# AMReX-Fluids/IAMR

Hardware: AMD Instinct MI355X
Metric: cells-advanced/sec (higher is better)
Workload: dtype f64; 1 GPU; TaylorGreen 3D single level, one 256^3 box per GPU in a 1x1x1 arrangement (256x256x256 cells), periodic, nu=1e-4 cfl=0.7 Godunov_PLM be_cn_theta=0.5, full NavierStokes::advance per step

## Files before the change

### iamr_amd/csrc/diffusion.hip

```cpp
#include "operators.h"
#include "launch.h"

namespace iamrx {

void scale_by(MultiFab& y, const MultiFab& x, int xcomp, int ng, bool divide);

namespace {
void scale_comp(MultiFab& y, int ycomp, const MultiFab& x, int xcomp, int ng, bool divide)
{
    const FabD *yt = y.d_tab, *xt = x.d_tab;
    for_each(*y.layout, cell_type(), ng, Context::get().stream, [=] __device__(int i, int j, int k, int f) {
        const double x = xt[f](i, j, k, xcomp);
        if (!divide) yt[f](i, j, k, ycomp) *= x;
        else if (x != 0.0 || yt[f](i, j, k, ycomp) != 0.0) yt[f](i, j, k, ycomp) /= x;
    });
}
void crse_soln(MultiFab& out, const MultiFab& Sc, int sigma, int rho_comp, bool over_rho)
{
    out.define(Sc.layout, cell_type(), 1, 0);
    MultiFab::Copy(out, Sc, sigma, 0, 1, 0);
    if (over_rho) scale_comp(out, 0, Sc, rho_comp, 0, true);
}
}

// ... 82 lines not shown
    MultiFab Rhs(layout, cell_type(), 3, 0);
    const bool want_flux = tflux != nullptr && tflux[0] != nullptr;
    TensorFlux fx{{want_flux ? tflux[0] : nullptr, want_flux ? tflux[1] : nullptr, want_flux ? tflux[2] : nullptr}, 0.0, false};
    if (want_flux) for (int d = 0; d < 3; ++d) tflux[d]->setVal(0.0);
    MultiFab cdata;
    TensorCF cf{&cdata, crse ? crse->cgeom : nullptr, crse ? crse->ratio : 2};
    const bool from_visc = theta != 1.0 && !want_flux && visc_old_term;
    if (!from_visc && theta != 1.0) {
        IAMRX_ASSERT(U_old && U_old->ngrow >= 1);
        MultiFab Soln0(layout, cell_type(), 3, 1);
        MultiFab::Copy(Soln0, *U_old, Xvel, 0, 3, 1);
        if (crse) { cdata.define(crse->crse_old->layout, cell_type(), 3, 0); MultiFab::Copy(cdata, *crse->crse_old, Xvel, 0, 3, 0); }
        fx.fac = 1.0 - theta; fx.add = false;
        tensor_apply(g, Rhs, Soln0, 0.0, -(1.0 - theta) * dt, nullptr, eta_n, bc_visc, 3, crse ? &cf : nullptr, want_flux ? &fx : nullptr);
    } else if (!from_visc) Rhs.setVal(0.0);
    {
        const FabD *nt = U_new.d_tab, *ot = U_old ? U_old->d_tab : nullptr, *rt = Rhs.d_tab, *ht = rho_half.d_tab;
        const FabD* vt = from_visc ? visc_old_term->d_tab : nullptr;
        const double va = (1.0 - theta) * dt;
        const bool mom = rho_flag == 3;
        IAMRX_ASSERT(!mom || ot);
        for_each(*layout, cell_type(), 0, Context::get().stream, [=] __device__(int i, int j, int k, int f) {
            const double r = mom ? ot[f](i, j, k, rho_comp) : ht[f](i, j, k, 0);
            for (int n = 0; n < 3; ++n) {
                const double un = nt[f](i, j, k, n) * r;
                nt[f](i, j, k, n) = un;
                double rr;
                if (vt) { const double v = vt[f](i, j, k, n); rr = va * v + 0.0 * v; }
                else rr = rt[f](i, j, k, n);
                rt[f](i, j, k, n) = rr + un;
            }
        });
    }
    double avg = 0.0;
    double rn3[3];
    Rhs.norm0_comps(0, 3, 0, rn3);
    for (int n = 0; n < 3; ++n) avg += (1.0 / 3.0) * rn3[n];
    const double tol_abs = visc_tol * avg;
    if (fill_new) fill_new(U_new);
    MultiFab Soln, acoef;
    Soln.view_of(U_new, Xvel, 3);
    if (rho_flag == 3) acoef.view_of(U_new, rho_comp, 1);
    else acoef.view_of(rho_half, 0, 1);
    MGOpts vo = o;
    vo.maxorder = 2;
    if (crse) { cdata.define(crse->crse_new->layout, cell_type(), 3, 0); MultiFab::Copy(cdata, *crse->crse_new, Xvel, 0, 3, 0); }
    fx.fac = theta; fx.add = true;
    MGStats st = tensor_solve(g, Soln, Rhs, 1.0, theta * dt, &acoef, eta_np1, bc_visc, 3, visc_tol, tol_abs, vo, crse ? &cf : nullptr, want_flux ? &fx : nullptr);
    return st;
}

// ... 59 lines not shown
```

### iamr_amd/csrc/k_abec.hip

```cpp
#include "kernels.h"
#include "launch.h"
#include <map>
#include <array>
#include <cstring>
#include <vector>
#include <algorithm>

namespace iamrx {

struct CfC1 { double c1[3][3]; double c2[3][3], c3[3][3]; int maxorder; int maintain; };

__device__ __forceinline__ void cf_maintain(const FabD& phi, const FabD& cfm, const BoxD& b, const CfC1& t, int i, int j, int k, double pnew)
{
    const int idx[3] = {i, j, k};
    for (int d = 0; d < 3; ++d) {
        const int NX = min(b.len(d) + 1, t.maxorder);
        if (NX < 2) continue;
        const int target = NX == 2 ? 1 : 2;
        for (int side = 0; side < 2; ++side) {
            const int s = side == 0 ? 1 : -1, f = side == 0 ? b.lo[d] : b.hi[d];
            if ((idx[d] - f) * s + 1 != target) continue;
            int g[3] = {i, j, k};
            g[d] = f - s;
            if (cfm(g[0], g[1], g[2]) != 1.0) continue;
// ... 860 lines not shown
    }
    return true;
}

static bool abec_sig_on() { return tune("ABEC_SIG", 1) != 0; }

AbecLevel abec_level(const AbecCoef& c, const MultiFab& phi, int rhs_ngrow, int nbc, const DomainBC* bcs, bool has_cf, bool finest)
{
    AbecLevel lv;
    const Layout& l = *phi.layout;
    lv.boxes = &l.boxes; lv.nlocal = l.nlocal();
    for (int d = 0; d < 3; ++d) lv.max_len[d] = l.max_len[d];
    lv.ncomp = phi.ncomp; lv.phi_ngrow = phi.ngrow; lv.rhs_ngrow = rhs_ngrow;
    lv.sig = c.sig != nullptr; lv.sig_ngrow = c.sig ? c.sig->ngrow : 0;
    lv.has_a = c.a && c.alpha != 0.0; lv.a_ngrow = c.a ? c.a->ngrow : 0;
    lv.b_uniform = c.b_uniform != 0; lv.tensor_eta = c.tensor_eta != 0; lv.tensor = c.tensor != 0; lv.b_ncomp = c.b[0]->ncomp;
    lv.nbc = nbc; lv.bcs = bcs; lv.has_cf = has_cf; lv.finest = finest;
    return lv;
}

static bool rb_shape_ok(const BoxD& b, int nx) { return (nx == 128 || nx == 256) && b.len(0) == nx && b.len(1) >= 16 && b.len(2) >= 16; }
static bool rb_walls_covered(const Geometry& g, const AbecLevel& lv)
{
    if (g.periodic[0] && g.periodic[1] && g.periodic[2]) return true;
    if (!lv.bcs || lv.nbc < 1) return false;
    for (int n = 0; n < lv.ncomp; ++n) { RbBC r; if (!rb_make_bc(g, lv.bcs[n < lv.nbc ? n : 0], r)) return false; }
    return true;
}
static bool box_spans(const Geometry& g, const BoxD& b, int min_len)
{
    for (int d = 0; d < 3; ++d) if (b.lo[d] != g.domain.lo[d] || b.hi[d] != g.domain.hi[d] || b.len(d) < min_len) return false;
// ... 1572 lines not shown
        const FabD fa = ft[f], ca = ct[f];
        const int c[3] = {i, j, k};
        for (int n = 0; n < nc; ++n) {
            double s = 0.0;
            for (int rb = 0; rb < 2; ++rb)
                for (int ra = 0; ra < 2; ++ra) {
                    int q[3];
                    q[dir] = 2 * c[dir]; q[da] = 2 * c[da] + ra; q[db] = 2 * c[db] + rb;
                    s += fa(q[0], q[1], q[2], n);
                }
            ca(i, j, k, n) = s * 0.25;
        }
    });
}

void abec_flux(const Geometry& g, const AbecCoef& c, const MultiFab& phi, MultiFab* const flux[3], MultiFab* const add_to[3])
{
    if (phi.nlocal() == 0) return;
    const FabD* pt = phi.d_tab;
    const int nc = phi.ncomp;
    for (int d = 0; d < 3; ++d) {
        const double fac = c.beta / g.dx[d];
        const FabD* bt = c.b[d]->d_tab;
        const int bnc = c.b[d]->ncomp;
        const FabD* ft = flux && flux[d] ? flux[d]->d_tab : nullptr;
        const FabD* ut = add_to && add_to[d] ? add_to[d]->d_tab : nullptr;
        for_each(*phi.layout, face_type(d), 0, Context::get().stream, [=] __device__(int i, int j, int k, int f) {
            const FabD p = pt[f], b = bt[f];
            int m[3] = {i, j, k}; m[d] -= 1;
            for (int n = 0; n < nc; ++n) {
// ... 4 lines not shown
        });
    }
}

void mac_divergence(const Geometry& g, MultiFab& div, const MultiFab* const umac[3])
{
    if (div.nlocal() == 0) return;
    const FabD *dt = div.d_tab, *ut = umac[0]->d_tab, *vt = umac[1]->d_tab, *wt = umac[2]->d_tab;
    const double dx = g.dx[0], dy = g.dx[1], dz = g.dx[2];
    for_each(*div.layout, cell_type(), 0, Context::get().stream, [=] __device__(int i, int j, int k, int f) {
        const FabD u = ut[f], v = vt[f], w = wt[f];
        dt[f](i, j, k, 0) = (u(i + 1, j, k) - u(i, j, k)) / dx + (v(i, j + 1, k) - v(i, j, k)) / dy + (w(i, j, k + 1) - w(i, j, k)) / dz;
    });
}

void mac_rhs(const Geometry& g, MultiFab& rhs, const MultiFab* const umac[3], const MultiFab* S)
{
    if (rhs.nlocal() == 0) return;
    const FabD *rt = rhs.d_tab, *ut = umac[0]->d_tab, *vt = umac[1]->d_tab, *wt = umac[2]->d_tab;
    const FabD* st = S ? S->d_tab : nullptr;
    const double dx = g.dx[0], dy = g.dx[1], dz = g.dx[2];
    for_each(*rhs.layout, cell_type(), 0, Context::get().stream, [=] __device__(int i, int j, int k, int f) {
        const FabD u = ut[f], v = vt[f], w = wt[f];
        const double div = (u(i + 1, j, k) - u(i, j, k)) / dx + (v(i, j + 1, k) - v(i, j, k)) / dy + (w(i, j, k + 1) - w(i, j, k)) / dz;
        double r = -div;
        if (st) r += st[f](i, j, k, 0);
        rt[f](i, j, k, 0) = r;
    });
}

void mac_bcoef(MultiFab* const b[3], const MultiFab& rho, int rho_comp, double scale)
{
    if (rho.nlocal() == 0) return;
    const FabD* rt = rho.d_tab;
    for (int d = 0; d < 3; ++d) {
        const FabD* bt = b[d]->d_tab;
        for_each(*rho.layout, face_type(d), 0, Context::get().stream, [=] __device__(int i, int j, int k, int f) {
            const FabD r = rt[f];
            int m[3] = {i, j, k}; m[d] -= 1;
            const double rf = 0.5 * (r(m[0], m[1], m[2], rho_comp) + r(i, j, k, rho_comp));
            bt[f](i, j, k, 0) = scale / rf;
        });
    }
}
// ... 29 lines not shown
```

### iamr_amd/csrc/k_basic.hip

```cpp
#include "kernels.h"
#include "launch.h"
#include <algorithm>

namespace iamrx {

__global__ void __launch_bounds__(256) k_fill(double* __restrict__ p, size_t n, double v)
{
    size_t i = (size_t)blockIdx.x * 256 + threadIdx.x;
    const size_t stride = (size_t)gridDim.x * 256;
    for (; i < n; i += stride) p[i] = v;
}

void launch_fill(double* p, size_t n, double v, hipStream_t s)
{
    if (n == 0) return;
    size_t nb = (n + 255) / 256;
    if (nb > 4096) nb = 4096;
    hipLaunchKernelGGL(k_fill, dim3((unsigned)nb), dim3(256), 0, s, p, n, v);
}

__global__ void __launch_bounds__(256) k_copy_plan(const CopyDesc* __restrict__ descs, const FabD* __restrict__ src,
                                                   const FabD* __restrict__ dst, int scomp, int dcomp, int nc, int add)
{
    const CopyDesc cd = descs[blockIdx.y];
// ... 507 lines not shown
    for_each_2ph(*y.layout, y.type, ng, nc, Context::get().stream,
        [=] __device__(int i, int j, int k, int f, int n) { return yt[f](i, j, k, ycomp + n) + a * xt[f](i, j, k, xcomp + n); },
        [=] __device__(int i, int j, int k, int f, int n, double v) { yt[f](i, j, k, ycomp + n) = v; });
}

void mf_add_scalar(MultiFab& y, double a, int comp, int nc, int ng)
{
    if (!y.base) return;
    const FabD* yt = y.d_tab;
    for_each(*y.layout, y.type, ng, Context::get().stream, [=] __device__(int i, int j, int k, int f) {
        const FabD yy = yt[f];
        for (int n = 0; n < nc; ++n) yy(i, j, k, comp + n) += a;
    });
}

void mf_mult(MultiFab& y, double a, int comp, int nc, int ng)
{
    trace_blas_site("mult", y.layout ? y.layout->local_cells() * nc : 0);
    if (!y.base) return;
    const FabD* yt = y.d_tab;
    for_each_2ph(*y.layout, y.type, ng, nc, Context::get().stream,
        [=] __device__(int i, int j, int k, int f, int n) { return yt[f](i, j, k, comp + n) * a; },
        [=] __device__(int i, int j, int k, int f, int n, double v) { yt[f](i, j, k, comp + n) = v; });
}

__global__ void __launch_bounds__(256) k_mult_shell(const BoxD* __restrict__ boxes, const FabD* __restrict__ yt, int t0, int t1, int t2, int ng, int comp, int nc, double a)
{
    const int fab = blockIdx.y;
    BoxD b = boxes[fab];
    b.hi[0] += t0; b.hi[1] += t1; b.hi[2] += t2;
// ... 145 lines not shown
```

### iamr_amd/csrc/kernels.h

```cpp
#pragma once
#include "core.h"
#include "mf.h"

namespace iamrx {

void launch_fill(double* p, size_t n, double v, hipStream_t s);
void launch_copy_plan(const CopyDesc* d, int nd, long maxpts, const FabD* src, const FabD* dst, int scomp, int dcomp, int nc, hipStream_t s, bool add = false);
void launch_pack(const CopyDesc* d, int nd, long maxpts, const FabD* src, double* buf, long pts_total, int scomp, int nc, hipStream_t s);
void launch_unpack(const CopyDesc* d, int nd, long maxpts, const FabD* dst, const double* buf, long pts_total, int dcomp, int nc, hipStream_t s, bool add = false);
void launch_copy_plan_w(const CopyDesc* d, const int2* w, int nw, const FabD* src, const FabD* dst, int scomp, int dcomp, int nc, hipStream_t s, bool add);
void launch_pack_w(const CopyDesc* d, const int2* w, int nw, const FabD* src, double* buf, long pts_total, int scomp, int nc, hipStream_t s);
void launch_unpack_w(const CopyDesc* d, const int2* w, int nw, const FabD* dst, const double* buf, long pts_total, int dcomp, int nc, hipStream_t s, bool add);
double reduce_norm0(const MultiFab& mf, int comp, int nc, int ng, bool global = false);
void reduce_norm0_comps(const MultiFab& mf, int comp, int nc, int ng, double* out, bool global = false);
void reduce_minmax(const MultiFab& mf, int comp, int ng, double& mn, double& mx, bool global = true);
double reduce_sum_unique(const MultiFab& mf, int comp, const Geometry& g, bool global = false);
void reduce_sum_integrated(const MultiFab& S, int rho_comp, int trac_comp, const MultiFab* cov, double out[3]);
constexpr int SUM_COMPS_MAX = 8;
void reduce_sum_comps(const MultiFab& mf, int n, const int* comps, const MultiFab* cov, double* out);
void reduce_dots(int nout, const MultiFab* const* x, const MultiFab* const* y, int comp, int nc, const Geometry& g, double* out, bool local = false);
void reduce_dots_dev(int nout, const MultiFab* const* x, const MultiFab* const* y, int comp, int nc, const Geometry& g, double* d_out, bool local = false);
enum { PROBE_NODAL_GS4 = 0, PROBE_ABEC_GSRB = 1, PROBE_GOD_Z = 2, PROBE_PRED_Z = 3, PROBE_COUNT = 4 };
void kernel_probe_start(int which, long min_points, int stride);
void kernel_probe_stop(int which, double* total_ms, long* launches);
void kernel_probes_pause(bool on);
bool kernel_probe_begin(int which, long points);
void kernel_probe_end(int which);
void gs4_probe_start(long min_nodes, int stride);
void gs4_probe_stop(double* total_ms, long* launches);
void mf_lincomb(MultiFab& dst, double a, const MultiFab& x, double b, const MultiFab& y, int comp, int nc, int ng);
void mf_saxpy(MultiFab& y, double a, const MultiFab& x, int xcomp, int ycomp, int nc, int ng);
void mf_add_scalar(MultiFab& y, double a, int comp, int nc, int ng);
void mf_mult(MultiFab& y, double a, int comp, int nc, int ng);
void mf_mult_ghosts(MultiFab& y, double a, int comp, int nc, int ng);
void dense_check_cover(const char* who, const Geometry& g, const Layout& lay);
void dense_pack(const Geometry& g, const MultiFab& S, int comp, double* dst, bool cplx);
void dense_pack_imag(const Geometry& g, const MultiFab& S, int comp, double* dst);
void dense_gather(const Geometry& g, const MultiFab& S, int comp, double* R);
bool dense_needs_gather(const MultiFab& S);
void dense_unpack(const Geometry& g, MultiFab& S, int comp, const double* src, double scale);

void stats_accumulate(MultiFab& avg, const MultiFab& S, int vcomp, double dt_avg, double t_sum, bool fluct);
void stats_derive_vel_avg(MultiFab& out, int ocomp, const MultiFab& avg, double t_mean, double t_fluct);

constexpr int PROFILE_NQ = 14;
struct ProfileLevel { const MultiFab* S; const MultiFab* cov; const Geometry* g; };
int profile_nbins(const Geometry& g0, int dir, int bin_level);
// ... 179 lines not shown
bool abec_gsrb_rb_cf_ok(const Geometry& g, const AbecCoef& c, const MultiFab& phi);
bool abec_gsrb_rb_nbr_ok(const Geometry& g, const AbecCoef& c, const MultiFab& phi, const MultiFab& rhs, int nbc, const DomainBC* bcs);
bool abec_gsrb_rb_nbr_level_ok(const Geometry& g, const Layout& l, int ncomp, bool sig_form, bool has_a, int nbc, const DomainBC* bcs);
void abec_gsrb_fused(const Geometry& g, const AbecCoef& c, const MultiFab& phi_in, MultiFab& phi_out, const MultiFab& rhs, double omega,
                     const DomainBC* bcs, int nbc);
void abec_residual(const Geometry& g, const AbecCoef& c, MultiFab& out, const MultiFab& phi, const MultiFab* rhs, double* norm_out = nullptr);
bool abec_bottom_device_ok(const Geometry& g, const Layout& l, const DomainBC* bcs, int nbc, int ncomp, bool cf = false);
void abec_bottom_solve(const Geometry& g, const AbecCoef& c, MultiFab& cor, const MultiFab& res, const DomainBC& bc, bool singular,
                       double eps_rel, int maxiter, int nub, int nuf, double omega, int* d_iters, const CfTab* cftab = nullptr);
void abec_apply_domain_bc(const Geometry& g, MultiFab& phi, const DomainBC& bc, bool inhomog, const MultiFab* bcval, int comp0 = 0, int ncomp = -1);
void abec_apply_domain_bc_percomp(const Geometry& g, MultiFab& phi, const DomainBC* bcs, int ncomp, bool inhomog, const MultiFab* bcval);
void cc_restrict(MultiFab& crse, const MultiFab& fine);
void cc_prolong_add(MultiFab& fine, const MultiFab& crse);
void face_avgdown(MultiFab& crse, const MultiFab& fine, int dir);
void abec_flux(const Geometry& g, const AbecCoef& c, const MultiFab& phi, MultiFab* const flux[3], MultiFab* const add_to[3]);
void mac_rhs(const Geometry& g, MultiFab& rhs, const MultiFab* const umac[3], const MultiFab* S);
void mac_bcoef(MultiFab* const b[3], const MultiFab& rho, int rho_comp, double scale);
void mac_divergence(const Geometry& g, MultiFab& div, const MultiFab* const umac[3]);

void godunov_extrap_vel_to_faces(const Geometry& g, const MultiFab& vel, const MultiFab* force, MultiFab* const umac[3],
                                 double dt, const BCRec* bc, bool use_forces_in_trans, int scheme = 0);
void godunov_compute_aofs(const Geometry& g, MultiFab& aofs, int acomp, const MultiFab& S, int ncomp, const MultiFab* force,
                          const MultiFab* divu, MultiFab* const umac[3], const int* iconserv, double dt, const BCRec* bc,
                          bool is_velocity, bool use_forces_in_trans, MultiFab* const edge_out[3], MultiFab* const flux_out[3], int scheme = 0);


struct NodalImages { bool on = false; int refl = 0; };
bool nodal_residual(const Geometry& g, MultiFab& out, const MultiFab& x, const MultiFab& sig, const MultiFab* rhs, double* norm_out = nullptr,
                    const NodalImages& img = NodalImages());
void nodal_gs_color(const Geometry& g, MultiFab& x, const MultiFab& rhs, const MultiFab& sig, int color, const MultiFab* dmask = nullptr);
struct NodalLevel {
    const std::vector<BoxD>* boxes = nullptr;
// ... 66 lines not shown
```

### iamr_amd/csrc/macproj.hip

```cpp
#include "operators.h"
#include "launch.h"

namespace iamrx {

LayoutP merged_solve_layout(const Geometry& g, const LayoutP& l)
{
    if (!l || l->replicated || l->total_cells() != g.domain.npts()) return nullptr;
    LayoutP ml = coalesce_layout(l);
    return (ml->id != l->id && ml->boxes.size() < l->boxes.size()) ? ml : nullptr;
}

MGStats mlmg_mac_solve(const Geometry& g, MultiFab* const umac[3], const MultiFab& rho, int rho_comp, const MultiFab* S,
                       MultiFab& mac_phi, double rhs_scale, const DomainBC& bc, double mac_tol, double mac_abs_tol,
                       const MGOpts& opts, MultiFab* const fluxes[3], const MultiFab* cphi, const Geometry* cgeom, int ratio)
{
    LayoutP layout = mac_phi.layout;
    if (!cgeom) {
        if (LayoutP ml = merged_solve_layout(g, layout)) {
            MultiFab um_m[3], fl_m[3], rho_m(ml, cell_type(), 1, std::min(rho.ngrow, 1)), phi_m(ml, cell_type(), 1, mac_phi.ngrow), S_m;
            MultiFab *ump[3], *flp[3];
            for (int d = 0; d < 3; ++d) {
                um_m[d].define(ml, face_type(d), 1, 0); relayout_copy(um_m[d], *umac[d], 1); ump[d] = &um_m[d];
                if (fluxes) { fl_m[d].define(ml, face_type(d), 1, 0); flp[d] = &fl_m[d]; }
            }
            relayout_copy(rho_m, rho, 1, rho_comp, 0);
            relayout_copy(phi_m, mac_phi, 1);
            if (S) { S_m.define(ml, cell_type(), 1, 0); relayout_copy(S_m, *S, 1); }
            MGStats st = mlmg_mac_solve(g, ump, rho_m, 0, S ? &S_m : nullptr, phi_m, rhs_scale, bc, mac_tol, mac_abs_tol, opts, fluxes ? flp : nullptr,
                                        nullptr, nullptr, ratio);
            relayout_copy(mac_phi, phi_m, 1);
            for (int d = 0; d < 3; ++d) { relayout_copy(*umac[d], um_m[d], 1); if (fluxes) relayout_copy(*fluxes[d], fl_m[d], 1); }
            return st;
        }
    }
    MultiFab bcoef[3];
    MultiFab* bp[3];
    const MultiFab* bcp[3];
    for (int d = 0; d < 3; ++d) { bcoef[d].define(layout, face_type(d), 1, 0); bp[d] = &bcoef[d]; bcp[d] = &bcoef[d]; }
    mac_bcoef(bp, rho, rho_comp, 1.0 / rhs_scale);

    MultiFab rhs(layout, cell_type(), 1, 0);
    const MultiFab* um[3] = {umac[0], umac[1], umac[2]};
    mac_rhs(g, rhs, um, S);

    CellMG mg(g, layout, 1, bc, opts);
    mg.setScalars(0.0, 1.0);
    mg.setBCoeffs(bcp);
    if (rho.ngrow >= 1) mg.setBCoeffsFromCell(&rho, rho_comp, 1.0 / rhs_scale);
    if (cgeom) mg.setCoarseFineBC(cphi, *cgeom, ratio);
    mg.prepare();
    MGStats st = mg.solve(mac_phi, rhs, mac_tol, mac_abs_tol);
    mg.fluxes(mac_phi, fluxes, umac);
    return st;
}

MGStats mac_sync_solve(const Geometry& g, FluxRegister& mr, const MultiFab& rho_half, double dt, LayoutP fine_layout, int ratio,
                       MultiFab* const Ucorr[3], MultiFab& mac_sync_phi, const DomainBC& bc, double tol, double abs_tol, const MGOpts& opts,
                       const Geometry* cgeom, int cratio)
{
    LayoutP layout = mac_sync_phi.layout;
    MultiFab Rhs(layout, cell_type(), 1, 0);
    Rhs.setVal(0.0);
    mr.Reflux(Rhs, g.dx[0] * g.dx[1] * g.dx[2], -1.0, 0, 0, 1);
    {
        MultiFab fz(fine_layout, cell_type(), 1, 0);
        fz.setVal(0.0);
// ... 14 lines not shown
```

### iamr_amd/csrc/mf.h

```cpp
#pragma once
#include <functional>
#include "core.h"
#include <vector>
#include <memory>
#include <map>
#include <array>

namespace iamrx {

enum class ReduceOp { Sum, Max, Min };

struct Message {
    int peer;
    double* dev_ptr;
    size_t count;
};

struct Comm {
    int rank = 0, nranks = 1;
    virtual ~Comm() = default;
    virtual void allreduce(double* host_vals, int n, ReduceOp op) { (void)host_vals; (void)n; (void)op; }
    virtual void allreduce_device(double* dev_vals, int n, ReduceOp op, hipStream_t s) { (void)dev_vals; (void)n; (void)op; (void)s; }
    virtual void exchange(const std::vector<Message>& sends, const std::vector<Message>& recvs, hipStream_t s)
    {
// ... 64 lines not shown
    void mark() { IAMRX_ASSERT(next < ev.size()); IAMRX_HIP_CHECK(hipEventRecord(ev[next++], Context::get().stream)); }
    static void mark(PassTimer* t) { if (t) t->mark(); }
    void finish(float* ms)
    {
        IAMRX_ASSERT(next == ev.size());
        IAMRX_HIP_CHECK(hipEventSynchronize(ev.back()));
        for (size_t q = 0; q + 1 < ev.size(); ++q) IAMRX_HIP_CHECK(hipEventElapsedTime(&ms[q], ev[q], ev[q + 1]));
        next = 0;
    }
};

double tune(const char* key, double dflt);
double tune_by_name(const char* key, double dflt);
void trace_blas_site(const char* what, long points);
void tuning_set(const char* key, double value);
void tuning_load_environment();

struct ProfScope {
    static bool enabled;
    bool on;
    std::string key;
    double t0 = 0.0;
    explicit ProfScope(const char* name);
    ~ProfScope();
};
#define PROF_NEXT(var, name) do { (var).reset(); (var) = std::make_unique<::iamrx::ProfScope>(name); } while (0)
void scope_profile_enable(bool on, bool reset);
std::string scope_profile_report();

void register_layout_evictor(std::function<void(uint64_t)> f);
// ... 144 lines not shown
```

### iamr_amd/csrc/mf.hip

```cpp
#include "mf.h"
#include <climits>
#include <array>
#include <execinfo.h>
#include <dlfcn.h>
#include <chrono>
#include <functional>
#include <tuple>
#include "launch.h"
#include "kernels.h"
#include <algorithm>
#include <cstring>
#include <atomic>

namespace iamrx {

Context& Context::get()
{
    static Context c;
    return c;
}

void Context::init(int dev)
{
    tuning_load_environment();
// ... 209 lines not shown
{
    size_t i = ((uintptr_t)key >> 2) & (kTuneSlots - 1);
    for (int probe = 0; probe < 16; ++probe, i = (i + 1) & (kTuneSlots - 1)) {
        TuneSlot& t = g_tune_slots[i];
        if (t.key == key && t.ver == g_tune_version) return t.set ? t.val : dflt;
        if (t.key == nullptr || t.ver != g_tune_version) {
            auto& m = tuning_map();
            auto it = m.find(key);
            t.key = key; t.ver = g_tune_version; t.set = it != m.end(); t.val = t.set ? it->second : 0.0;
            return t.set ? t.val : dflt;
        }
    }
    return tune_by_name(key, dflt);
}
void tuning_set(const char* key, double value) { tuning_map()[key] = value; ++g_tune_version; }

bool ProfScope::enabled = false;
namespace {
struct ScopeStat { double ms = 0.0; long calls = 0; };
std::map<std::string, ScopeStat>& scope_stats() { static auto* m = new std::map<std::string, ScopeStat>(); return *m; }
std::vector<std::string>& scope_stack() { static auto* v = new std::vector<std::string>(); return *v; }
double now_ms() { return std::chrono::duration<double, std::milli>(std::chrono::steady_clock::now().time_since_epoch()).count(); }
}
ProfScope::ProfScope(const char* name) : on(enabled)
{
    if (!on) return;
    auto& st = scope_stack();
    key = st.empty() ? std::string(name) : st.back() + "/" + name;
    st.push_back(key);
    Context::get().sync();
// ... 888 lines not shown
```

### iamr_amd/csrc/mlmg.h

```cpp
#pragma once
#include <functional>
#include "mf.h"
#include "kernels.h"
#include <vector>
#include <memory>

namespace iamrx {

inline bool mg_stalled_at_floor(const std::vector<double>& hist, double r0, double target, bool fast)
{
    const size_t n = hist.size();
    if (n == 0 || !(hist[n - 1] <= 10.0 * target)) return false;
    if (n >= 4 && hist[n - 1] > 0.9 * hist[n - 4]) return true;
    if (!fast || n < 2) return false;
    const double last = hist[n - 1] / hist[n - 2];
    double best = 1.0, prev = r0;
    for (size_t i = 0; i + 1 < n; ++i) { if (prev > 0.0) best = std::min(best, hist[i] / prev); prev = hist[i]; }
    return last > 0.5 && best < 0.2;
}


struct MGOpts {
    int nu1 = 2, nu2 = 2, nuf = 8, nub = 0;
    int max_iters = 200;
// ... 77 lines not shown

class CellMG {
public:
    CellMG(const Geometry& g, LayoutP layout, int ncomp, const DomainBC& bc, const MGOpts& o);
    void setScalars(double alpha, double beta) { m_alpha = alpha; m_beta = beta; }
    void setACoeffs(const MultiFab* a) { m_a0 = a; }
    void setBCoeffs(const MultiFab* const b[3]) { for (int d = 0; d < 3; ++d) m_b0[d] = b[d]; }
    void setBCoeffsFromCell(const MultiFab* sig, int comp, double scale) { m_sig = sig; m_sig_comp = comp; m_sig_scale = scale; }
    void setTensor(bool t) { m_tensor = t; }
    void setTensorEta(bool t) { m_tensor_eta = t; }
    void setDomainBCs(const DomainBC* bcs, int n) { m_bcn.assign(bcs, bcs + n); }
    void setCoarseFineBC(const MultiFab* crse, const Geometry& cgeom, int ratio) { m_cf = true; m_crse = crse; m_cgeom = cgeom; m_ratio = ratio; }
    void prepare();
    void prepareBoundary();
    void fillBoundaryData(MultiFab& phi);
    MGStats solve(MultiFab& phi, const MultiFab& rhs, double rtol, double atol);
    void apply(MultiFab& out, MultiFab& phi);
    void fluxes(MultiFab& phi, MultiFab* const flux[3], MultiFab* const add_to[3]);
    int nlevels() const { return (int)m_lev.size(); }
    AbecCoef coef(int l) const;
    AbecCoef smoother_coef(int l) const;
    const Geometry& geom(int l) const { return m_lev[l].g; }
    void applyBC(int l, MultiFab& phi, bool inhomog, const MultiFab* bcval, bool corners = true);
    void smooth(int l, bool skip_fill, bool cf_ghosts_current = false, bool sol_is_zero = false);
    void smooth_n(int l, int nsweeps, bool skip_first_fill, bool sol_is_zero = false, MultiFab* acc = nullptr);
    void vcycle(MGStats& st);
    MultiFab& res(int l) { return m_lev[l].res; }
    MultiFab& cor(int l) { return m_lev[l].cor; }

private:
    struct Level : MGLevel {
        MultiFab a, b[3];
        MultiFab cor, res, rescor;
        MultiFab buf;
        AbecSmoothPlan plan;
        AbecLegPlan legs;
        MultiFab cfm;
        CfTab cftab;
    };
    int bicgstab(int l, MultiFab& sol, const MultiFab& rhs, double eps_rel, double eps_abs, int& niters);
    void bottom_solve(MGStats& st);
    template <class Sweep> void pingpong(MultiFab& sol, MultiFab& buf, int nsweeps, bool sol_is_zero, MultiFab* acc, Sweep sweep);
    bool tail_fused() const;
    void cf_bcval(MultiFab& bcval);
    void prepare_cf(int l);
    void subtract_mean(int l, MultiFab& mf);
    Geometry m_g;
    int m_ncomp;
    std::vector<DomainBC> m_bcn;
    MGOpts m_o;
    double m_alpha = 0.0, m_beta = 1.0;
    const MultiFab* m_a0 = nullptr;
    const MultiFab* m_b0[3] = {nullptr, nullptr, nullptr};
    bool m_buni = false;
    bool m_buni_coarse = false;
    double m_bu[3] = {0.0, 0.0, 0.0};
    const MultiFab* m_sig = nullptr;
    int m_sig_comp = 0;
    double m_sig_scale = 1.0;
    bool m_tensor = false;
    bool m_tensor_eta = false;
    bool m_singular = false;
    bool m_bottom_dev = false;
    MultiFab* m_acc = nullptr;
    bool m_acc_done = false;
    bool m_bottom_direct = false;
    const double* m_dB = nullptr;
    std::shared_ptr<double> m_dBh;
// ... 59 lines not shown
```

### iamr_amd/csrc/mlmg.hip

```cpp
#include "mlmg.h"
#include "krylov.h"
#include "launch.h"
#include <chrono>
#include <cmath>

namespace iamrx {

void parallel_copy(MultiFab& dst, const MultiFab& src, int scomp, int dcomp, int nc, int src_ng, int dst_ng, const Geometry* periodic_geom, bool add);

CycleTimer& cycle_timer() { static CycleTimer t; return t; }

long mg_agglomeration_cells() { return (long)tune("MG_AGGLOMERATE_CELLS", 2097152.0); }

bool mg_agglomerate_level(const Layout& c)
{
    if (c.replicated || c.total_cells() > mg_agglomeration_cells()) return false;
    if (Context::get().comm->nranks > 1) return true;
    return c.boxes.size() > 1 && tune("MG_AGG_SINGLE_RANK", 1) != 0;
}

bool mg_slab_level(const Geometry& g, const Layout& l, int min_width, bool slab_problem)
{
    if (!slab_problem && tune("MG_SLAB", 0) == 0) return false;
    if (!g.periodic[1] || g.domain.lo[1] != 0 || g.domain.hi[1] != 1) return false;
// ... 90 lines not shown
    if (!m_cf) return;
    Level& L = m_lev[l];
    double loc[3];
    for (int d = 0; d < 3; ++d) loc[d] = 0.5 * m_ratio * m_g.dx[d];
    L.cftab = cf_make_tab(loc, L.g.dx, m_o.maxorder);
    L.cfm.define(L.layout, cell_type(), 1, l == 0 ? 2 : 1);
    cf_build_mask(L.g, L.cfm);
}

void CellMG::prepareBoundary()
{
    m_lev.resize(1);
    prepare_cf(0);
}

void CellMG::prepare()
{
    ProfScope ps_prof_("cmg_prepare");
    IAMRX_ASSERT(m_b0[0] && m_b0[1] && m_b0[2]);
    m_singular = !(m_alpha != 0.0 && m_a0);
    for (int d = 0; d < 3; ++d)
        for (auto& b : m_bcn) if (!m_g.periodic[d] && (b.lo[d] == lo_dirichlet || b.hi[d] == lo_dirichlet)) m_singular = false;
    if (m_cf) m_singular = false;
    m_buni = false;
    if (!m_sig && m_b0[0]->ncomp == 1) {
        m_buni = true;
        for (int d = 0; d < 3 && m_buni; ++d) {
            if (m_b0[d]->uniform_marked) {
                m_bu[d] = m_b0[d]->uniform_value;
                if (tune("CHECK_UNIFORM", 0) != 0) {
                    double v = 0.0;
                    if (!mf_uniform_value(*m_b0[d], &v) || v != m_bu[d]) throw Error("iamrx: an array marked uniform is not (MultiFab::mark_uniform)");
                }
            }
            else if (m_b0[d]->varying_marked) m_buni = false;
            else m_buni = mf_uniform_value(*m_b0[d], &m_bu[d]);
        }
    }
    m_buni_coarse = m_buni && tune("MG_COARSE_UNIFORM", 1) != 0;
    m_dd_sweeps = 0;
    const bool dd_on = tune("MG_DIAG_SHORTCUT", 1) != 0;
    if (dd_on && m_alpha > 0.0 && m_beta > 0.0 && m_a0 && m_o.fixed_iters <= 0 && m_o.max_coarsening_level > 0) {
        double bmax = 0.0;
        for (int d = 0; d < 3; ++d) bmax = std::max(bmax, m_buni ? std::fabs(m_bu[d]) : m_b0[d]->norm0(0, m_b0[d]->ncomp, 0));
        if (m_tensor_eta) bmax *= 4.0 / 3.0;
        MultiFab inv(m_lev[0].layout, cell_type(), 1, 0);
        {
            const FabD *it = inv.d_tab, *at = m_a0->d_tab;
            for_each(*m_lev[0].layout, cell_type(), 0, Context::get().stream, [=] __device__(int i, int j, int k, int f) {
                const double a = at[f](i, j, k);
                it[f](i, j, k) = a > 0.0 ? 1.0 / a : 1.e300;
            });
        }
        const double ainv = inv.norm0(0, 1, 0);
        double q = 0.0;
        for (int d = 0; d < 3; ++d) q += 2.0 / (m_g.dx[d] * m_g.dx[d]);
        q *= m_beta * bmax;
        const double jac = ainv < 1.e299 ? q / (m_alpha / ainv + q) : 1.0;
        if (jac < 0.2) m_dd_sweeps = jac < 0.05 ? 2 : (jac < 0.12 ? 3 : 4);
        m_dd_rho = m_dd_sweeps > 0 ? std::max(jac * jac, 1.e-6) : 0.0;
        const int dd_force = (int)tune("MG_DD_SWEEPS", 0);
        if (m_dd_sweeps > 0 && dd_force > 0) { m_dd_sweeps = dd_force; m_dd_rho = 0.0; }
        if (m_o.verbose) printf("iamrx MLMG: Jacobi bound %.3e -> %d sweeps per cycle\n", jac, m_dd_sweeps);
    }
    m_lev.resize(1);
    while (m_dd_sweeps == 0 && (int)m_lev.size() <= m_o.max_coarsening_level) {
        Level& f = m_lev.back();
        if (m_o.device_bottom && !m_tensor && !m_o.bottom_smoother_only && abec_bottom_device_ok(f.g, *f.layout, m_bcn.data(), (int)m_bcn.size(), m_ncomp, m_cf)) break;
        Level c;
// ... 30 lines not shown
            if (L.agg) L.tmp_d.define(L.dist, cell_type(), m_ncomp, 0);
            if (L.slab) L.vres.define(L.virt, cell_type(), m_ncomp, 0);
            auto coarsen_into = [&](MultiFab& dst, IndexType t, int nc, const std::function<void(MultiFab&)>& op) {
                MultiFab dist_arr, v;
                if (L.agg) dist_arr.define(L.dist, t, nc, 0);
                if (L.slab) v.define(L.virt, t, nc, 0);
                mg_restrict_to(L, dst, dist_arr, v, op);
            };
            if (m_a0) {
                L.a.define(L.layout, cell_type(), 1, 0);
                coarsen_into(L.a, cell_type(), 1, [&](MultiFab& c) { cc_restrict(c, *fc.a); });
            }
            for (int d = 0; d < 3; ++d) {
                MultiFab b3;
                const MultiFab* fb = fc.b[d];
                if (l == 1 && m_tensor_eta && !m_buni_coarse) { b3.define(m_lev[0].layout, face_type(d), 3, 0); tensor_bcoef(b3, *fc.b[d], d); fb = &b3; }
                L.b[d].define(L.layout, face_type(d), fb->ncomp, 0);
                coarsen_into(L.b[d], face_type(d), fb->ncomp, [&](MultiFab& c) { face_avgdown(c, *fb, d); });
            }
        }
        L.plan = abec_smooth_plan(L.g, abec_level(coef(l), L.cor, L.res.ngrow, (int)m_bcn.size(), m_bcn.data(), m_cf, l == 0));
    }
    for (int l = 0; l < nl; ++l) {
        Level& L = m_lev[l];
        L.legs = AbecLegPlan();
        if (l < 1 || l + 1 >= nl || m_dd_sweeps > 0) continue;
        const Level& C = m_lev[l + 1];
        L.legs = abec_leg_plan(L.g, abec_level(coef(l), L.cor, L.res.ngrow, (int)m_bcn.size(), m_bcn.data(), m_cf, false), l, m_o.nu1, m_o.nu2,
                               L.slab || C.slab, C.agg);
    }
    if (nl >= 2 && m_lev[nl - 2].legs.on && tail_fused()) m_lev[nl - 2].legs.on = false;
    for (int l = 0; l < nl; ++l) {
        Level& L = m_lev[l];
        if (L.legs.on && (!L.buf.defined() || L.buf.ngrow != L.cor.ngrow)) L.buf.define(L.layout, cell_type(), m_ncomp, L.cor.ngrow);
    }
    bottom_direct_prepare();
}
// ... 377 lines not shown
        MultiFab bcval(m_lev[0].layout, cell_type(), m_ncomp, 1);
        MultiFab::Copy(bcval, phi, 0, 0, m_ncomp, 1);
        cf_bcval(bcval);
        applyBC(0, phi, true, &bcval);
    } else applyBC(0, phi, true, nullptr);
}

void CellMG::apply(MultiFab& out, MultiFab& phi)
{
    fillBoundaryData(phi);
    level_residual(m_lev[0].g, coef(0), out, phi, nullptr);
}

void CellMG::fluxes(MultiFab& phi, MultiFab* const flux[3], MultiFab* const add_to[3])
{
    abec_flux(m_lev[0].g, coef(0), phi, flux, add_to);
}

MGStats CellMG::solve(MultiFab& phi, const MultiFab& rhs_in, double rtol, double atol)
{
    ProfScope ps_prof_("cmg_solve");
    auto& ctx = Context::get();
    MGStats st;
    st.nlevels = (int)m_lev.size();
    Level& L0 = m_lev[0];
    const int nc = m_ncomp;
    MultiFab rhs_own;
    if (m_singular) {
        rhs_own.define(L0.layout, cell_type(), nc, 0);
        MultiFab::Copy(rhs_own, rhs_in, 0, 0, nc, 0);
        subtract_mean(0, rhs_own);
    }
    const MultiFab& rhs = m_singular ? rhs_own : rhs_in;
    const bool has_bcdata = m_cf || !(L0.g.periodic[0] && L0.g.periodic[1] && L0.g.periodic[2]);
    MultiFab bcval_own;
    if (has_bcdata) {
        bcval_own.define(L0.layout, cell_type(), nc, 1);
        MultiFab::Copy(bcval_own, phi, 0, 0, nc, 1);
        cf_bcval(bcval_own);
    }
    const MultiFab* bcvp = has_bcdata ? &bcval_own : nullptr;

    applyBC(0, phi, true, bcvp);
    level_residual(L0.g, coef(0), L0.res, phi, &rhs, &st.resnorm0);
    st.rhsnorm0 = rhs.norm0(0, nc, 0);
    const double max_norm = st.rhsnorm0 >= st.resnorm0 ? st.rhsnorm0 : st.resnorm0;
    if (!std::isfinite(max_norm)) throw Error("iamrx MLMG: the right-hand side or the initial residual is not finite");
    const double res_target = std::max(atol, std::max(rtol, 1.e-16) * max_norm);
    st.resnorm = st.resnorm0;
    if (m_o.verbose) printf("iamrx MLMG: rhs %.6e resid0 %.6e target %.3e levels %d\n", st.rhsnorm0, st.resnorm0, res_target, st.nlevels);
    double vc_ms = 0.0;
    hipGraphExec_t vc_exec = nullptr;
    cycle_timer().used = 0;
    if (m_bottom_dev) IAMRX_HIP_CHECK(hipMemsetAsync(mg_bottom_iters_dev(), 0, sizeof(int), ctx.stream));
    if (m_o.fixed_iters <= 0 && st.resnorm0 <= res_target) st.converged = 1;
    else {
        const int maxit = m_o.fixed_iters > 0 ? m_o.fixed_iters : m_o.max_iters;
        for (int iter = 0; iter < maxit; ++iter) {
            if (m_singular && (has_bcdata || tune("MG_RES_MEAN", 0) != 0)) subtract_mean(0, L0.res);
            if (m_dd_sweeps > 0 && m_dd_rho > 0.0 && st.resnorm > 0.0) {
// ... 50 lines not shown
```

Baseline: 499.8 million cells/s.

## Fuse MAC solve setup: compute face coefficients from cell density and fold norms into kernels

The MAC projection now skips materialising face b-coefficient arrays by default, deriving them on the fly from cell density in the smoother, in a new coarse-level avgdown and in a new flux kernel. The rhs construction also computes its sum inside the same kernel, and the singular mean-subtraction is done in place together with the max-norm. Elsewhere, the tensor-diffusion RHS loop and the a-inverse computation fuse their norm reductions instead of running separate passes. This removes several full-grid allocations, copies and reduction passes, at the cost of more code paths, recomputed divisions, and a fallback that materialises arrays when the fused smoother path cannot use them.

```diff
diff --git a/iamr_amd/csrc/diffusion.hip b/iamr_amd/csrc/diffusion.hip
--- a/iamr_amd/csrc/diffusion.hip
+++ b/iamr_amd/csrc/diffusion.hip
@@ -120,27 +120,30 @@
         fx.fac = 1.0 - theta; fx.add = false;
         tensor_apply(g, Rhs, Soln0, 0.0, -(1.0 - theta) * dt, nullptr, eta_n, bc_visc, 3, crse ? &cf : nullptr, want_flux ? &fx : nullptr);
     } else if (!from_visc) Rhs.setVal(0.0);
+    double rn3[3];
     {
         const FabD *nt = U_new.d_tab, *ot = U_old ? U_old->d_tab : nullptr, *rt = Rhs.d_tab, *ht = rho_half.d_tab;
         const FabD* vt = from_visc ? visc_old_term->d_tab : nullptr;
         const double va = (1.0 - theta) * dt;
         const bool mom = rho_flag == 3;
         IAMRX_ASSERT(!mom || ot);
-        for_each(*layout, cell_type(), 0, Context::get().stream, [=] __device__(int i, int j, int k, int f) {
+        reduce_max_f<3>(*layout, cell_type(), 0, [=] __device__(int i, int j, int k, int f, double (&m)[3]) {
             const double r = mom ? ot[f](i, j, k, rho_comp) : ht[f](i, j, k, 0);
+#pragma unroll
             for (int n = 0; n < 3; ++n) {
                 const double un = nt[f](i, j, k, n) * r;
                 nt[f](i, j, k, n) = un;
                 double rr;
                 if (vt) { const double v = vt[f](i, j, k, n); rr = va * v + 0.0 * v; }
                 else rr = rt[f](i, j, k, n);
-                rt[f](i, j, k, n) = rr + un;
+                rr += un;
+                rt[f](i, j, k, n) = rr;
+                const double a = norm_term(rr);
+                m[n] = a > m[n] ? a : m[n];
             }
-        });
+        }, rn3);
     }
     double avg = 0.0;
-    double rn3[3];
-    Rhs.norm0_comps(0, 3, 0, rn3);
     for (int n = 0; n < 3; ++n) avg += (1.0 / 3.0) * rn3[n];
     const double tol_abs = visc_tol * avg;
     if (fill_new) fill_new(U_new);
diff --git a/iamr_amd/csrc/k_abec.hip b/iamr_amd/csrc/k_abec.hip
--- a/iamr_amd/csrc/k_abec.hip
+++ b/iamr_amd/csrc/k_abec.hip
@@ -898,7 +898,7 @@
     lv.ncomp = phi.ncomp; lv.phi_ngrow = phi.ngrow; lv.rhs_ngrow = rhs_ngrow;
     lv.sig = c.sig != nullptr; lv.sig_ngrow = c.sig ? c.sig->ngrow : 0;
     lv.has_a = c.a && c.alpha != 0.0; lv.a_ngrow = c.a ? c.a->ngrow : 0;
-    lv.b_uniform = c.b_uniform != 0; lv.tensor_eta = c.tensor_eta != 0; lv.tensor = c.tensor != 0; lv.b_ncomp = c.b[0]->ncomp;
+    lv.b_uniform = c.b_uniform != 0; lv.tensor_eta = c.tensor_eta != 0; lv.tensor = c.tensor != 0; lv.b_ncomp = c.b[0] ? c.b[0]->ncomp : 1;
     lv.nbc = nbc; lv.bcs = bcs; lv.has_cf = has_cf; lv.finest = finest;
     return lv;
 }
@@ -2501,6 +2501,69 @@
     });
 }
 
+void mac_bcoef_avgdown(MultiFab& crse, const MultiFab& rho, int rho_comp, double scale, int dir)
+{
+    if (crse.nlocal() == 0) return;
+    const FabD *rt = rho.d_tab, *ct = crse.d_tab;
+    const int d1 = (dir + 1) % 3, d2 = (dir + 2) % 3;
+    const int da = d1 < d2 ? d1 : d2, db = d1 < d2 ? d2 : d1;
+    for_each(*crse.layout, face_type(dir), 0, Context::get().stream, [=] __device__(int i, int j, int k, int f) {
+        const FabD r = rt[f];
+        const int c[3] = {i, j, k};
+        double s = 0.0;
+        for (int rb = 0; rb < 2; ++rb)
+            for (int ra = 0; ra < 2; ++ra) {
+                int q[3], m[3];
+                q[dir] = 2 * c[dir]; q[da] = 2 * c[da] + ra; q[db] = 2 * c[db] + rb;
+                m[0] = q[0]; m[1] = q[1]; m[2] = q[2]; m[dir] -= 1;
+                const double rf = 0.5 * (r(m[0], m[1], m[2], rho_comp) + r(q[0], q[1], q[2], rho_comp));
+                s += scale / rf;
+            }
+        ct[f](i, j, k, 0) = s * 0.25;
+    });
+}
+
+void abec_flux_sig(const Geometry& g, double beta, const MultiFab& rho, int rho_comp, double scale, const MultiFab& phi, MultiFab* const flux[3],
+                   MultiFab* const add_to[3])
+{
+    IAMRX_ASSERT(phi.ncomp == 1 && phi.ngrow >= 1 && rho.ngrow >= 1);
+    if (phi.nlocal() == 0) return;
+    const FabD *pt = phi.d_tab, *rt = rho.d_tab;
+    const BoxD* boxes = phi.layout->d_boxes;
+    const double fx = beta / g.dx[0], fy = beta / g.dx[1], fz = beta / g.dx[2];
+    const FabD* f0 = flux && flux[0] ? flux[0]->d_tab : nullptr;
+    const FabD* f1 = flux && flux[1] ? flux[1]->d_tab : nullptr;
+    const FabD* f2 = flux && flux[2] ? flux[2]->d_tab : nullptr;
+    const FabD* u0 = add_to && add_to[0] ? add_to[0]->d_tab : nullptr;
+    const FabD* u1 = add_to && add_to[1] ? add_to[1]->d_tab : nullptr;
+    const FabD* u2 = add_to && add_to[2] ? add_to[2]->d_tab : nullptr;
+    for_each(*phi.layout, node_type(), 0, Context::get().stream, [=] __device__(int i, int j, int k, int f) {
+        const BoxD b = boxes[f];
+        const bool in0 = i <= b.hi[0], in1 = j <= b.hi[1], in2 = k <= b.hi[2];
+        if ((in0 ? 0 : 1) + (in1 ? 0 : 1) + (in2 ? 0 : 1) >= 2) return;
+        const FabD p = pt[f], r = rt[f];
+        const double p0 = p(i, j, k, 0), r0 = r(i, j, k, rho_comp);
+        if (in1 && in2) {
+            const double bf = scale / (0.5 * (r(i - 1, j, k, rho_comp) + r0));
+            const double fl = -fx * bf * (p0 - p(i - 1, j, k, 0));
+            if (f0) f0[f](i, j, k, 0) = fl;
+            if (u0) u0[f](i, j, k, 0) += fl;
+        }
+        if (in0 && in2) {
+            const double bf = scale / (0.5 * (r(i, j - 1, k, rho_comp) + r0));
+            const double fl = -fy * bf * (p0 - p(i, j - 1, k, 0));
+            if (f1) f1[f](i, j, k, 0) = fl;
+            if (u1) u1[f](i, j, k, 0) += fl;
+        }
+        if (in0 && in1) {
+            const double bf = scale / (0.5 * (r(i, j, k - 1, rho_comp) + r0));
+            const double fl = -fz * bf * (p0 - p(i, j, k - 1, 0));
+            if (f2) f2[f](i, j, k, 0) = fl;
+            if (u2) u2[f](i, j, k, 0) += fl;
+        }
+    });
+}
+
 void abec_flux(const Geometry& g, const AbecCoef& c, const MultiFab& phi, MultiFab* const flux[3], MultiFab* const add_to[3])
 {
     if (phi.nlocal() == 0) return;
@@ -2535,20 +2598,6 @@
     });
 }
 
-void mac_rhs(const Geometry& g, MultiFab& rhs, const MultiFab* const umac[3], const MultiFab* S)
-{
-    if (rhs.nlocal() == 0) return;
-    const FabD *rt = rhs.d_tab, *ut = umac[0]->d_tab, *vt = umac[1]->d_tab, *wt = umac[2]->d_tab;
-    const FabD* st = S ? S->d_tab : nullptr;
-    const double dx = g.dx[0], dy = g.dx[1], dz = g.dx[2];
-    for_each(*rhs.layout, cell_type(), 0, Context::get().stream, [=] __device__(int i, int j, int k, int f) {
-        const FabD u = ut[f], v = vt[f], w = wt[f];
-        const double div = (u(i + 1, j, k) - u(i, j, k)) / dx + (v(i, j + 1, k) - v(i, j, k)) / dy + (w(i, j, k + 1) - w(i, j, k)) / dz;
-        double r = -div;
-        if (st) r += st[f](i, j, k, 0);
-        rt[f](i, j, k, 0) = r;
-    });
-}
 
 void mac_bcoef(MultiFab* const b[3], const MultiFab& rho, int rho_comp, double scale)
 {
diff --git a/iamr_amd/csrc/k_basic.hip b/iamr_amd/csrc/k_basic.hip
--- a/iamr_amd/csrc/k_basic.hip
+++ b/iamr_amd/csrc/k_basic.hip
@@ -545,6 +545,68 @@
     });
 }
 
+double mf_add_scalar_norm0(MultiFab& y, double a, int comp, int ng)
+{
+    const FabD* yt = y.d_tab;
+    double out = 0.0;
+    reduce_max_f<1>(*y.layout, y.type, ng, [=] __device__(int i, int j, int k, int f, double (&m)[1]) {
+        double v = yt[f](i, j, k, comp);
+        v += a;
+        yt[f](i, j, k, comp) = v;
+        const double t = norm_term(v);
+        m[0] = t > m[0] ? t : m[0];
+    }, &out);
+    return out;
+}
+
+template <bool SUM>
+__global__ void __launch_bounds__(256) k_mac_rhs(Tiling t, const BoxD* __restrict__ boxes, const FabD* __restrict__ rt, const FabD* __restrict__ ut,
+                                                 const FabD* __restrict__ vt, const FabD* __restrict__ wt, const FabD* __restrict__ st,
+                                                 double dx, double dy, double dz, double* __restrict__ partials)
+{
+    const int fab = tile_fab(t);
+    const BoxD b = boxes[fab];
+    int i, j, k0, k1;
+    double s = 0.0;
+    if (tile_ijk(t, b, i, j, k0, k1)) {
+        const FabD u = ut[fab], v = vt[fab], w = wt[fab], rr = rt[fab];
+        for (int k = k0; k <= k1; ++k) {
+            const double div = (u(i + 1, j, k) - u(i, j, k)) / dx + (v(i, j + 1, k) - v(i, j, k)) / dy + (w(i, j, k + 1) - w(i, j, k)) / dz;
+            double r = -div;
+            if (st) r += st[fab](i, j, k, 0);
+            rr(i, j, k, 0) = r;
+            if (SUM) s += r;
+        }
+    }
+    if (SUM) {
+        s = block_reduce<0>(s);
+        if (threadIdx.x == 0) partials[(size_t)blockIdx.y * gridDim.x + blockIdx.x] = s;
+    }
+}
+
+void mac_rhs(const Geometry& g, MultiFab& rhs, const MultiFab* const umac[3], const MultiFab* S, double* sum)
+{
+    auto& ctx = Context::get();
+    const bool global = !rhs.layout->replicated;
+    if (rhs.nlocal() == 0) {
+        if (sum) *sum = (global && ctx.comm->nranks > 1) ? finish_to_host(0, 1, 0, true) : 0.0;
+        return;
+    }
+    Tiling t = level_tiling(*rhs.layout, cell_type(), 0, 8, true);
+    dim3 gr = t.grid();
+    const int np = (int)(gr.x * gr.y);
+    const FabD* st = S ? S->d_tab : nullptr;
+    if (!sum) {
+        hipLaunchKernelGGL((k_mac_rhs<false>), gr, Tiling::block(), 0, ctx.stream, t, rhs.layout->d_boxes, rhs.d_tab, umac[0]->d_tab, umac[1]->d_tab,
+                           umac[2]->d_tab, st, g.dx[0], g.dx[1], g.dx[2], (double*)nullptr);
+        return;
+    }
+    ctx.ensure_scratch((size_t)np + 16);
+    hipLaunchKernelGGL((k_mac_rhs<true>), gr, Tiling::block(), 0, ctx.stream, t, rhs.layout->d_boxes, rhs.d_tab, umac[0]->d_tab, umac[1]->d_tab,
+                       umac[2]->d_tab, st, g.dx[0], g.dx[1], g.dx[2], ctx.d_scratch);
+    *sum = finish_to_host(0, 1, np, global);
+}
+
 void mf_mult(MultiFab& y, double a, int comp, int nc, int ng)
 {
     trace_blas_site("mult", y.layout ? y.layout->local_cells() * nc : 0);
diff --git a/iamr_amd/csrc/kernels.h b/iamr_amd/csrc/kernels.h
--- a/iamr_amd/csrc/kernels.h
+++ b/iamr_amd/csrc/kernels.h
@@ -31,6 +31,7 @@
 void mf_lincomb(MultiFab& dst, double a, const MultiFab& x, double b, const MultiFab& y, int comp, int nc, int ng);
 void mf_saxpy(MultiFab& y, double a, const MultiFab& x, int xcomp, int ycomp, int nc, int ng);
 void mf_add_scalar(MultiFab& y, double a, int comp, int nc, int ng);
+double mf_add_scalar_norm0(MultiFab& y, double a, int comp, int ng);
 void mf_mult(MultiFab& y, double a, int comp, int nc, int ng);
 void mf_mult_ghosts(MultiFab& y, double a, int comp, int nc, int ng);
 void dense_check_cover(const char* who, const Geometry& g, const Layout& lay);
@@ -240,8 +241,11 @@
 void cc_prolong_add(MultiFab& fine, const MultiFab& crse);
 void face_avgdown(MultiFab& crse, const MultiFab& fine, int dir);
 void abec_flux(const Geometry& g, const AbecCoef& c, const MultiFab& phi, MultiFab* const flux[3], MultiFab* const add_to[3]);
-void mac_rhs(const Geometry& g, MultiFab& rhs, const MultiFab* const umac[3], const MultiFab* S);
+void mac_rhs(const Geometry& g, MultiFab& rhs, const MultiFab* const umac[3], const MultiFab* S, double* sum = nullptr);
 void mac_bcoef(MultiFab* const b[3], const MultiFab& rho, int rho_comp, double scale);
+void mac_bcoef_avgdown(MultiFab& crse, const MultiFab& rho, int rho_comp, double scale, int dir);
+void abec_flux_sig(const Geometry& g, double beta, const MultiFab& rho, int rho_comp, double scale, const MultiFab& phi, MultiFab* const flux[3],
+                   MultiFab* const add_to[3]);
 void mac_divergence(const Geometry& g, MultiFab& div, const MultiFab* const umac[3]);
 
 void godunov_extrap_vel_to_faces(const Geometry& g, const MultiFab& vel, const MultiFab* force, MultiFab* const umac[3],
diff --git a/iamr_amd/csrc/macproj.hip b/iamr_amd/csrc/macproj.hip
--- a/iamr_amd/csrc/macproj.hip
+++ b/iamr_amd/csrc/macproj.hip
@@ -15,9 +15,10 @@
                        const MGOpts& opts, MultiFab* const fluxes[3], const MultiFab* cphi, const Geometry* cgeom, int ratio)
 {
     LayoutP layout = mac_phi.layout;
+    if (rho.ngrow < 1) throw Error("iamrx mlmg_mac_solve: the density needs one filled ghost layer");
     if (!cgeom) {
         if (LayoutP ml = merged_solve_layout(g, layout)) {
-            MultiFab um_m[3], fl_m[3], rho_m(ml, cell_type(), 1, std::min(rho.ngrow, 1)), phi_m(ml, cell_type(), 1, mac_phi.ngrow), S_m;
+            MultiFab um_m[3], fl_m[3], rho_m(ml, cell_type(), 1, 1), phi_m(ml, cell_type(), 1, mac_phi.ngrow), S_m;
             MultiFab *ump[3], *flp[3];
             for (int d = 0; d < 3; ++d) {
                 um_m[d].define(ml, face_type(d), 1, 0); relayout_copy(um_m[d], *umac[d], 1); ump[d] = &um_m[d];
@@ -33,23 +34,24 @@
             return st;
         }
     }
-    MultiFab bcoef[3];
-    MultiFab* bp[3];
-    const MultiFab* bcp[3];
-    for (int d = 0; d < 3; ++d) { bcoef[d].define(layout, face_type(d), 1, 0); bp[d] = &bcoef[d]; bcp[d] = &bcoef[d]; }
-    mac_bcoef(bp, rho, rho_comp, 1.0 / rhs_scale);
-
-    MultiFab rhs(layout, cell_type(), 1, 0);
-    const MultiFab* um[3] = {umac[0], umac[1], umac[2]};
-    mac_rhs(g, rhs, um, S);
-
+    const bool from_cell = tune("MAC_GLUE", 1) != 0;
+    MultiFab bcoef[3], rhs(layout, cell_type(), 1, 0);
     CellMG mg(g, layout, 1, bc, opts);
     mg.setScalars(0.0, 1.0);
-    mg.setBCoeffs(bcp);
-    if (rho.ngrow >= 1) mg.setBCoeffsFromCell(&rho, rho_comp, 1.0 / rhs_scale);
+    if (!from_cell) {
+        MultiFab* bp[3];
+        const MultiFab* bcp[3];
+        for (int d = 0; d < 3; ++d) { bcoef[d].define(layout, face_type(d), 1, 0); bp[d] = &bcoef[d]; bcp[d] = &bcoef[d]; }
+        mac_bcoef(bp, rho, rho_comp, 1.0 / rhs_scale);
+        mg.setBCoeffs(bcp);
+    }
+    mg.setBCoeffsFromCell(&rho, rho_comp, 1.0 / rhs_scale);
     if (cgeom) mg.setCoarseFineBC(cphi, *cgeom, ratio);
     mg.prepare();
-    MGStats st = mg.solve(mac_phi, rhs, mac_tol, mac_abs_tol);
+    const MultiFab* um[3] = {umac[0], umac[1], umac[2]};
+    double rhs_sum = 0.0;
+    mac_rhs(g, rhs, um, S, mg.singular() ? &rhs_sum : nullptr);
+    MGStats st = mg.solve_giving_rhs(mac_phi, rhs, mac_tol, mac_abs_tol, mg.singular() ? &rhs_sum : nullptr);
     mg.fluxes(mac_phi, fluxes, umac);
     return st;
 }
diff --git a/iamr_amd/csrc/mf.h b/iamr_amd/csrc/mf.h
--- a/iamr_amd/csrc/mf.h
+++ b/iamr_amd/csrc/mf.h
@@ -102,6 +102,7 @@
 double tune_by_name(const char* key, double dflt);
 void trace_blas_site(const char* what, long points);
 void tuning_set(const char* key, double value);
+void tuning_count(const char* key);
 void tuning_load_environment();
 
 struct ProfScope {
diff --git a/iamr_amd/csrc/mf.hip b/iamr_amd/csrc/mf.hip
--- a/iamr_amd/csrc/mf.hip
+++ b/iamr_amd/csrc/mf.hip
@@ -247,6 +247,7 @@
     return tune_by_name(key, dflt);
 }
 void tuning_set(const char* key, double value) { tuning_map()[key] = value; ++g_tune_version; }
+void tuning_count(const char* key) { tuning_map()[key] += 1.0; }
 
 bool ProfScope::enabled = false;
 namespace {
diff --git a/iamr_amd/csrc/mlmg.h b/iamr_amd/csrc/mlmg.h
--- a/iamr_amd/csrc/mlmg.h
+++ b/iamr_amd/csrc/mlmg.h
@@ -115,7 +115,9 @@
     void prepare();
     void prepareBoundary();
     void fillBoundaryData(MultiFab& phi);
-    MGStats solve(MultiFab& phi, const MultiFab& rhs, double rtol, double atol);
+    MGStats solve(MultiFab& phi, const MultiFab& rhs, double rtol, double atol) { return solve_on(phi, rhs, nullptr, rtol, atol, nullptr); }
+    MGStats solve_giving_rhs(MultiFab& phi, MultiFab& rhs, double rtol, double atol, const double* rhs_sum = nullptr) { return solve_on(phi, rhs, &rhs, rtol, atol, rhs_sum); }
+    bool singular() const { return m_singular; }
     void apply(MultiFab& out, MultiFab& phi);
     void fluxes(MultiFab& phi, MultiFab* const flux[3], MultiFab* const add_to[3]);
     int nlevels() const { return (int)m_lev.size(); }
@@ -139,6 +141,7 @@
         MultiFab cfm;
         CfTab cftab;
     };
+    MGStats solve_on(MultiFab& phi, const MultiFab& rhs_in, MultiFab* rhs_mine, double rtol, double atol, const double* rhs_sum);
     int bicgstab(int l, MultiFab& sol, const MultiFab& rhs, double eps_rel, double eps_abs, int& niters);
     void bottom_solve(MGStats& st);
     template <class Sweep> void pingpong(MultiFab& sol, MultiFab& buf, int nsweeps, bool sol_is_zero, MultiFab* acc, Sweep sweep);
@@ -153,6 +156,8 @@
     double m_alpha = 0.0, m_beta = 1.0;
     const MultiFab* m_a0 = nullptr;
     const MultiFab* m_b0[3] = {nullptr, nullptr, nullptr};
+    MultiFab m_b0_own[3];
+    void materialise_b();
     bool m_buni = false;
     bool m_buni_coarse = false;
     double m_bu[3] = {0.0, 0.0, 0.0};
diff --git a/iamr_amd/csrc/mlmg.hip b/iamr_amd/csrc/mlmg.hip
--- a/iamr_amd/csrc/mlmg.hip
+++ b/iamr_amd/csrc/mlmg.hip
@@ -128,10 +128,19 @@
     prepare_cf(0);
 }
 
+void CellMG::materialise_b()
+{
+    MultiFab* bp[3];
+    for (int d = 0; d < 3; ++d) { m_b0_own[d].define(m_lev[0].layout, face_type(d), 1, 0); bp[d] = &m_b0_own[d]; m_b0[d] = &m_b0_own[d]; }
+    mac_bcoef(bp, *m_sig, m_sig_comp, m_sig_scale);
+    tuning_count("MAC_GLUE_MATERIALISED");
+}
+
 void CellMG::prepare()
 {
     ProfScope ps_prof_("cmg_prepare");
-    IAMRX_ASSERT(m_b0[0] && m_b0[1] && m_b0[2]);
+    IAMRX_ASSERT((m_b0[0] && m_b0[1] && m_b0[2]) || (m_sig && !m_b0[0] && !m_b0[1] && !m_b0[2]));
+    if (!m_b0[0] && !(m_ncomp == 1 && !m_tensor && !m_tensor_eta && !(m_a0 && m_alpha != 0.0) && tune("ABEC_SIG", 1) != 0)) materialise_b();
     m_singular = !(m_alpha != 0.0 && m_a0);
     for (int d = 0; d < 3; ++d)
         for (auto& b : m_bcn) if (!m_g.periodic[d] && (b.lo[d] == lo_dirichlet || b.hi[d] == lo_dirichlet)) m_singular = false;
@@ -158,15 +167,15 @@
         double bmax = 0.0;
         for (int d = 0; d < 3; ++d) bmax = std::max(bmax, m_buni ? std::fabs(m_bu[d]) : m_b0[d]->norm0(0, m_b0[d]->ncomp, 0));
         if (m_tensor_eta) bmax *= 4.0 / 3.0;
-        MultiFab inv(m_lev[0].layout, cell_type(), 1, 0);
+        double ainv = 0.0;
         {
-            const FabD *it = inv.d_tab, *at = m_a0->d_tab;
-            for_each(*m_lev[0].layout, cell_type(), 0, Context::get().stream, [=] __device__(int i, int j, int k, int f) {
+            const FabD* at = m_a0->d_tab;
+            reduce_max_f<1>(*m_lev[0].layout, cell_type(), 0, [=] __device__(int i, int j, int k, int f, double (&m)[1]) {
                 const double a = at[f](i, j, k);
-                it[f](i, j, k) = a > 0.0 ? 1.0 / a : 1.e300;
-            });
-        }
-        const double ainv = inv.norm0(0, 1, 0);
+                const double v = norm_term(a > 0.0 ? 1.0 / a : 1.e300);
+                m[0] = v > m[0] ? v : m[0];
+            }, &ainv);
+        }
         double q = 0.0;
         for (int d = 0; d < 3; ++d) q += 2.0 / (m_g.dx[d] * m_g.dx[d]);
         q *= m_beta * bmax;
@@ -227,13 +236,21 @@
             for (int d = 0; d < 3; ++d) {
                 MultiFab b3;
                 const MultiFab* fb = fc.b[d];
+                if (!fb) {
+                    L.b[d].define(L.layout, face_type(d), 1, 0);
+                    coarsen_into(L.b[d], face_type(d), 1, [&](MultiFab& c) { mac_bcoef_avgdown(c, *m_sig, m_sig_comp, m_sig_scale, d); });
+                    if (d == 0) tuning_count("MAC_GLUE_LEVEL1");
+                    continue;
+                }
                 if (l == 1 && m_tensor_eta && !m_buni_coarse) { b3.define(m_lev[0].layout, face_type(d), 3, 0); tensor_bcoef(b3, *fc.b[d], d); fb = &b3; }
                 L.b[d].define(L.layout, face_type(d), fb->ncomp, 0);
                 coarsen_into(L.b[d], face_type(d), fb->ncomp, [&](MultiFab& c) { face_avgdown(c, *fb, d); });
             }
         }
         L.plan = abec_smooth_plan(L.g, abec_level(coef(l), L.cor, L.res.ngrow, (int)m_bcn.size(), m_bcn.data(), m_cf, l == 0));
-    }
+        if (l == 0 && !m_b0[0] && (L.plan.path == AbecSmoothPlan::FUSED_SHELL || (nl == 1 && m_bottom_dev))) materialise_b();
+    }
+    if (!m_b0[0]) tuning_count("MAC_GLUE_NO_ARRAYS");
     for (int l = 0; l < nl; ++l) {
         Level& L = m_lev[l];
         L.legs = AbecLegPlan();
@@ -641,10 +658,15 @@
 
 void CellMG::fluxes(MultiFab& phi, MultiFab* const flux[3], MultiFab* const add_to[3])
 {
+    if (m_sig && m_ncomp == 1 && (!m_b0[0] || tune("MAC_GLUE", 1) != 0)) {
+        abec_flux_sig(m_lev[0].g, m_beta, *m_sig, m_sig_comp, m_sig_scale, phi, flux, add_to);
+        tuning_count("MAC_GLUE_FLUX");
+        return;
+    }
     abec_flux(m_lev[0].g, coef(0), phi, flux, add_to);
 }
 
-MGStats CellMG::solve(MultiFab& phi, const MultiFab& rhs_in, double rtol, double atol)
+MGStats CellMG::solve_on(MultiFab& phi, const MultiFab& rhs_in, MultiFab* rhs_mine, double rtol, double atol, const double* rhs_sum)
 {
     ProfScope ps_prof_("cmg_solve");
     auto& ctx = Context::get();
@@ -653,12 +675,21 @@
     Level& L0 = m_lev[0];
     const int nc = m_ncomp;
     MultiFab rhs_own;
-    if (m_singular) {
+    const bool inplace = m_singular && rhs_mine;
+    if (m_singular && !inplace) {
         rhs_own.define(L0.layout, cell_type(), nc, 0);
         MultiFab::Copy(rhs_own, rhs_in, 0, 0, nc, 0);
-        subtract_mean(0, rhs_own);
-    }
-    const MultiFab& rhs = m_singular ? rhs_own : rhs_in;
+    }
+    const MultiFab& rhs = !m_singular ? rhs_in : (inplace ? rhs_in : rhs_own);
+    if (m_singular) {
+        MultiFab& w = inplace ? *rhs_mine : rhs_own;
+        const double ncell = (double)L0.g.domain.npts();
+        for (int n = 0; n < nc; ++n) {
+            const double s = (rhs_sum && nc == 1) ? *rhs_sum : w.sum_unique(L0.g, n);
+            const double m = mf_add_scalar_norm0(w, -s / ncell, n, 0);
+            st.rhsnorm0 = m > st.rhsnorm0 ? m : st.rhsnorm0;
+        }
+    }
     const bool has_bcdata = m_cf || !(L0.g.periodic[0] && L0.g.periodic[1] && L0.g.periodic[2]);
     MultiFab bcval_own;
     if (has_bcdata) {
@@ -670,7 +701,7 @@
 
     applyBC(0, phi, true, bcvp);
     level_residual(L0.g, coef(0), L0.res, phi, &rhs, &st.resnorm0);
-    st.rhsnorm0 = rhs.norm0(0, nc, 0);
+    if (!m_singular) st.rhsnorm0 = rhs.norm0(0, nc, 0);
     const double max_norm = st.rhsnorm0 >= st.resnorm0 ? st.rhsnorm0 : st.resnorm0;
     if (!std::isfinite(max_norm)) throw Error("iamrx MLMG: the right-hand side or the initial residual is not finite");
     const double res_target = std::max(atol, std::max(rtol, 1.e-16) * max_norm);
```

Result: faster. 508.4 million cells/s, median of 6 (+1.7%).
